# zengyan-97/X2-VLM

Hardware: AMD Instinct MI355X
Metric: image-text pairs/sec (fwd+bwd) X2VLM-base 224px bs=64/GPU (higher is better)
Workload: dtype bf16

## Files before the change

probes/nt_phase_times.py:

```python
import ctypes, importlib, os, sys
sys.path.insert(0, os.path.dirname(os.path.dirname(os.path.abspath(__file__))))
import torch
K = importlib.import_module("x2-vlm_amd.kernels")
lib = importlib.import_module("x2-vlm_amd._lib").lib()
assert hasattr(lib, "x2_probe_set_buffer"), "needs the probe build: X2VLM_HIP_LIB=probes/_probe/libx2vlm_hip_probe.so"
lib.x2_probe_set_buffer.argtypes, lib.x2_probe_set_buffer.restype = [ctypes.c_void_p], ctypes.c_int
dev = "cuda"
NSET = 12
SHAPES = [("vit qkv", 12608, 2304, 768, "bias"), ("vit dqkv", 12608, 768, 2304, "plain"), ("vit dfc1", 12608, 768, 3072, "plain"),
          ("vit fc2", 12608, 768, 3072, "lscale"), ("vit dproj", 12608, 768, 768, "plain"), ("fus xkv", 12608, 1536, 768, "bias"),
          ("vit fc1 (forced)", 12608, 3072, 768, "gelu"), ("vitL qkv", 18464, 3072, 1024, "bias"), ("vitL dfc1", 18464, 1024, 4096, "plain")]


def launch(kind, A, W, out, extra):
    if kind == "bias":
        K.gemm_nt(A, W, bias=extra["bias"], out=out)
    elif kind == "plain":
        K.gemm_nt(A, W, out=out)
    elif kind == "lscale":
        K.gemm_nt(A, W, bias=extra["bias"], gamma=extra["gamma"], resid=extra["resid"], out=out)
    elif kind == "gelu":
        K.gemm_nt(A, W, bias=extra["bias"], aux=extra["aux"], act=1, out=out)


for name, M, N, Kd, kind in SHAPES:
    f32 = kind == "lscale"
    As = [torch.randn(M, Kd, device=dev).bfloat16() for _ in range(NSET)]
    W = (torch.randn(N, Kd, device=dev) / Kd ** 0.5).bfloat16()
    outs = [torch.empty(M, N, device=dev, dtype=torch.float32 if f32 else torch.bfloat16) for _ in range(NSET)]
    extra = dict(bias=torch.randn(N, device=dev), gamma=torch.rand(N, device=dev), resid=torch.randn(M, N, device=dev) if f32 else None,
                 aux=torch.empty(M, N, device=dev, dtype=torch.bfloat16) if kind == "gelu" else None)
    lib.x2_tune(1, 3)
    nbuf = torch.zeros(4096 * 4, device=dev, dtype=torch.int64)
    for i in range(NSET):
        launch(kind, As[i], W, outs[i], extra)
    torch.cuda.synchronize()
    rows = []
    for rep in range(6):
        nbuf.zero_()
        lib.x2_probe_set_buffer(ctypes.c_void_p(nbuf.data_ptr()))
        launch(kind, As[rep % NSET], W, outs[rep % NSET], extra)
        torch.cuda.synchronize()
        lib.x2_probe_set_buffer(None)
        t = nbuf.view(-1, 4).cpu().double()
        t = t[t[:, 3] > 0] / 100.0
        t0 = t[:, 0].min()
        rows.append((t.shape[0], (t[:, 1] - t[:, 0]), (t[:, 2] - t[:, 1]), (t[:, 3] - t[:, 2]), float(t[:, 3].max() - t0),
                     float((t[:, 0] - t0).quantile(0.9))))
    lib.x2_tune(1, 0)
    n = rows[0][0]
    pro = torch.cat([r[1] for r in rows[1:]]); main = torch.cat([r[2] for r in rows[1:]]); epi = torch.cat([r[3] for r in rows[1:]])
    span = sum(r[4] for r in rows[1:]) / len(rows[1:])
    busy = float((pro.sum() + main.sum() + epi.sum()) / len(rows[1:])) / 256.0
    print("%-18s M=%6d N=%5d K=%5d %-6s | %4d wgs (%.2f rounds) | launch %6.1f us | prologue %5.2f (p90 %5.2f)  main %6.2f (p90 %6.2f)  epilogue %5.2f (p90 %5.2f) us"
          " | per CU: %.1f us busy = %.0f %% of the launch: prologue %.0f %%, main %.0f %%, epilogue %.0f %%; entry of the 90th percentile wg %+.1f us"
          % (name, M, N, Kd, kind, n, n / 256.0, span, pro.mean(), pro.quantile(0.9), main.mean(), main.quantile(0.9), epi.mean(), epi.quantile(0.9),
             busy, 100 * busy / span, 100 * float(pro.sum()) / float(pro.sum() + main.sum() + epi.sum()),
             100 * float(main.sum()) / float(pro.sum() + main.sum() + epi.sum()), 100 * float(epi.sum()) / float(pro.sum() + main.sum() + epi.sum()),
             rows[-1][5]))
```

x2-vlm_amd/csrc/gemm.hip:

```cpp
#include "x2_common.h"
#include <type_traits>

#define BM 128
#define BN 128
#define BK 64
#define TILE_BYTES (128 * 128)
#define STAGE_BYTES (2 * TILE_BYTES)
#define GEMM_LDS_BYTES (2 * STAGE_BYTES)

struct GemmNT {
  const bf16_t* A; const bf16_t* B; void* C;
  const float* bias; const float* gamma; const float* resid; bf16_t* aux;
  int M, N, K;
  int lda, ldb, ldc, ldr, ldaux;
  int act;
  int out_f32;
  int group_m;
  DropSpec drop;
  const uint32_t* drop_epoch;
  const float* rowscale;
  float* colsum;
  int dbg;
  int ksplit;
  const long* ce_labels;
  const float* ce_lse;
  const float* ce_g;
  const float* ce_stat;
  float* ce_part;
  float* ce_zlab;
  float ce_gscale;
  int ce_C;
  float* ce_sumz;
  float* ce_zign;
  long ce_ignore;
  float ce_ls;
  const float* ce_w;
};

__device__ __forceinline__ void tile_coords(int t, int tiles_m, int tiles_n, int gm, int& tm, int& tn) {
  const int gsz = gm * tiles_n, g = t / gsz, first = g * gm;
  const int rows = min(gm, tiles_m - first), r = t - g * gsz;
  tm = first + r % rows;
  tn = r / rows;
}

__device__ __forceinline__ void st16(void* p, u32x4 v, bool wt) {
  if (wt) asm volatile("global_store_dwordx4 %0, %1, off sc1\n\ts_nop 1" ::"v"(p), "v"(v) : "memory");
  else *reinterpret_cast<u32x4*>(p) = v;
}

#ifdef X2_PROBE
#define NT_DBG(p, bit) (((p).dbg & (bit)) != 0)
static __device__ unsigned long long* g_nt_probe = nullptr;
#define NT_STAMP(i) do { if (g_nt_probe && threadIdx.x == 0) g_nt_probe[(size_t)blockIdx.x * 4 + (i)] = wall_clock64(); } while (0)
#define NT_ABL_DECL(p) const bool abl_dma_ = NT_DBG(p, 32), abl_rd_ = NT_DBG(p, 64), abl_mm_ = NT_DBG(p, 128); bool rd_ = true
#define NT_ABL_NO_DMA(kt) if (abl_dma_ && (kt) >= 2) return
#define NT_ABL_NO_READ() if (!rd_) return
#define NT_ABL_NO_MFMA() if (abl_mm_) return
#define NT_ABL_STEP(kt) if (abl_rd_ && (kt) > 0) rd_ = false
#else
#define NT_ABL_DECL(p)
#define NT_ABL_NO_DMA(kt)
#define NT_ABL_NO_READ()
#define NT_ABL_NO_MFMA()
#define NT_ABL_STEP(kt)
#define NT_DBG(p, bit) false
#define NT_STAMP(i) do { } while (0)
#endif
typedef __attribute__((ext_vector_type(16))) float f32x16;
template <int TM>
__device__ __forceinline__ void epi_stage_half(f32x4 (&acc)[TM][4], int half, bool full, float* stg, int lane) {
  const int frow = lane & 15, fg = lane >> 4;
#pragma unroll
  for (int ii = 0; ii < 2; ++ii)
#pragma unroll
    for (int j = 0; j < 4; ++j)
      if (full || ii == 0) *reinterpret_cast<f32x4*>(stg + (ii * 16 + frow) * 68 + j * 16 + fg * 4) = acc[full ? half * 2 + ii : half * 2][j];
}
template <int RT>
__device__ __forceinline__ void epi_stage_half(f32x16 (&acc)[RT][2], int half, bool, float* stg, int lane) {
  const int row = lane & 31, h = lane >> 5;
#pragma unroll
  for (int tj = 0; tj < 2; ++tj)
#pragma unroll
    for (int g = 0; g < 4; ++g)
      *reinterpret_cast<f32x4*>(stg + row * 68 + tj * 32 + g * 8 + h * 4) =
          f32x4{acc[half][tj][4 * g], acc[half][tj][4 * g + 1], acc[half][tj][4 * g + 2], acc[half][tj][4 * g + 3]};
}
template <int V> struct EpiTraits {
  static constexpr bool generic = V == 4;
  static constexpr int act = V == 2 ? 1 : (V == 3 || V == 10) ? 2 : 0;
  static constexpr bool out_f32 = V == 1 || V == 5 || V == 6 || V == 7;
  static constexpr bool resid = V == 5 || V == 6;
  static constexpr bool scale = V == 6;
  static constexpr bool aux0 = false;
  static constexpr bool drop = V == 5;
  static constexpr bool colsum = false;
  static constexpr bool colparts = V == 10;
};
template <int TM, int VAR, class Acc>
__device__ __forceinline__ void nt_epilogue(const GemmNT& p, Acc& acc, char* smem, int wave, int lane, int mw0, int nw0, int prow = 0) {
  using E = EpiTraits<VAR>;
  const int act = E::generic ? p.act : E::act;
  const bool out_f32 = E::generic ? p.out_f32 != 0 : E::out_f32;
  const bool has_resid = E::generic ? p.resid != nullptr : E::resid;
  const bool has_scale = E::generic ? (p.gamma != nullptr || p.rowscale != nullptr) : E::scale;
  const bool has_aux0 = E::generic ? (p.act == 0 && p.aux != nullptr) : E::aux0;
  const bool has_drop = (E::generic || E::drop) ? p.drop.thr16 != 0 : false;
  const bool has_colsum = E::generic ? p.colsum != nullptr : (E::colsum && p.colsum != nullptr);
  float* stg = reinterpret_cast<float*>(smem) + wave * (32 * 68);
  const int er = lane >> 3, ec = (lane & 7) * 8;
  const int n = nw0 + ec;
  const bool nok = n < p.N;
  float bb[8], gg[8];
#pragma unroll
  for (int e = 0; e < 8; ++e) { bb[e] = 0.f; gg[e] = 1.f; }
  if (nok && p.bias) { const float4 b0 = *reinterpret_cast<const float4*>(p.bias + n), b1 = *reinterpret_cast<const float4*>(p.bias + n + 4);
    bb[0] = b0.x; bb[1] = b0.y; bb[2] = b0.z; bb[3] = b0.w; bb[4] = b1.x; bb[5] = b1.y; bb[6] = b1.z; bb[7] = b1.w; }
  if (nok && has_scale && p.gamma) { const float4 g0 = *reinterpret_cast<const float4*>(p.gamma + n), g1 = *reinterpret_cast<const float4*>(p.gamma + n + 4);
    gg[0] = g0.x; gg[1] = g0.y; gg[2] = g0.z; gg[3] = g0.w; gg[4] = g1.x; gg[5] = g1.y; gg[6] = g1.z; gg[7] = g1.w; }
  float cs[8] = {0.f, 0.f, 0.f, 0.f, 0.f, 0.f, 0.f, 0.f};
  const bool wt = NT_DBG(p, 16);
  const DropSpec drop_ = drop_at_epoch(p.drop, p.drop_epoch);
#pragma unroll
  for (int half = 0; half < (TM + 1) / 2; ++half) {
    const bool full = half * 2 + 1 < TM;
    float4 r0[4], r1[4];
    u32x4 pre[4];
    const int nc = nok ? n : 0;
    if (has_resid) {
#pragma unroll
      for (int rr = 0; rr < 4; ++rr) {
        if (!full && rr >= 2) continue;
        const int mc = min(mw0 + half * 32 + rr * 8 + er, p.M - 1);
        r0[rr] = *reinterpret_cast<const float4*>(p.resid + (size_t)mc * p.ldr + nc);
        r1[rr] = *reinterpret_cast<const float4*>(p.resid + (size_t)mc * p.ldr + nc + 4);
      }
    }
    if (act == 2) {
#pragma unroll
      for (int rr = 0; rr < 4; ++rr) {
        if (!full && rr >= 2) continue;
        const int mc = min(mw0 + half * 32 + rr * 8 + er, p.M - 1);
        pre[rr] = *reinterpret_cast<const u32x4*>(p.aux + (size_t)mc * p.ldaux + nc);
      }
    }
    epi_stage_half(acc, half, full, stg, lane);
#pragma unroll
    for (int rr = 0; rr < 4; ++rr) {
      if (!full && rr >= 2) continue;
      const int row = rr * 8 + er;
      const int m = mw0 + half * 32 + row;
      const float4 a0 = *reinterpret_cast<const float4*>(stg + row * 68 + ec), a1 = *reinterpret_cast<const float4*>(stg + row * 68 + ec + 4);
      if (m >= p.M || !nok) continue;
      float v[8] = {a0.x + bb[0], a0.y + bb[1], a0.z + bb[2], a0.w + bb[3], a1.x + bb[4], a1.y + bb[5], a1.z + bb[6], a1.w + bb[7]};
      if constexpr (VAR == 8) {
        const long lab = p.ce_labels[m];
        float mx = -INFINITY;
#pragma unroll
        for (int e = 0; e < 8; ++e) mx = n + e < p.ce_C ? fmaxf(mx, v[e]) : mx;
        mx = fmaxf(mx, __shfl_xor(mx, 1, 64)); mx = fmaxf(mx, __shfl_xor(mx, 2, 64)); mx = fmaxf(mx, __shfl_xor(mx, 4, 64));
        float se = 0.f;
#pragma unroll
        for (int e = 0; e < 8; ++e) {
          se += n + e < p.ce_C ? __expf(v[e] - mx) : 0.f;
          if ((long)(n + e) == lab) p.ce_zlab[m] = v[e];
        }
        se += __shfl_xor(se, 1, 64); se += __shfl_xor(se, 2, 64); se += __shfl_xor(se, 4, 64);
        if ((lane & 7) == 0) *reinterpret_cast<float2*>(p.ce_part + ((size_t)m * (p.N >> 6) + (nw0 >> 6)) * 2) = float2{mx, se};
        continue;
      }
      if constexpr (VAR == 11) {
        const long lab = p.ce_labels[m];
        float mx = -INFINITY, sz = 0.f;
#pragma unroll
        for (int e = 0; e < 8; ++e) { mx = n + e < p.ce_C ? fmaxf(mx, v[e]) : mx; sz += n + e < p.ce_C ? v[e] : 0.f; }
        mx = fmaxf(mx, __shfl_xor(mx, 1, 64)); mx = fmaxf(mx, __shfl_xor(mx, 2, 64)); mx = fmaxf(mx, __shfl_xor(mx, 4, 64));
        sz += __shfl_xor(sz, 1, 64); sz += __shfl_xor(sz, 2, 64); sz += __shfl_xor(sz, 4, 64);
        float se = 0.f;
#pragma unroll
        for (int e = 0; e < 8; ++e) {
          se += n + e < p.ce_C ? __expf(v[e] - mx) : 0.f;
          if ((long)(n + e) == lab) p.ce_zlab[m] = v[e];
          if ((long)(n + e) == p.ce_ignore) p.ce_zign[m] = v[e];
        }
        se += __shfl_xor(se, 1, 64); se += __shfl_xor(se, 2, 64); se += __shfl_xor(se, 4, 64);
        if ((lane & 7) == 0) {
          *reinterpret_cast<float2*>(p.ce_part + ((size_t)m * (p.N >> 6) + (nw0 >> 6)) * 2) = float2{mx, se};
          p.ce_sumz[(size_t)m * (p.N >> 6) + (nw0 >> 6)] = sz;
        }
        continue;
      }
      if constexpr (VAR == 12) {
        const long lab = p.ce_labels[m];
        const bool live = lab >= 0 && lab != p.ce_ignore;
        const float conf = 1.f - p.ce_ls, sm = p.ce_ls / (float)(p.ce_C - 2), qsum = conf + sm * (float)(p.ce_C - 2);
        const float sc = live ? p.ce_gscale * p.ce_g[0] * p.ce_w[m] / (p.ce_stat[1] + 1e-5f) : 0.f, l = p.ce_lse[m];
#pragma unroll
        for (int e = 0; e < 8; ++e) {
          const long c = n + e;
          const float q = c == lab ? conf : (c == p.ce_ignore ? 0.f : sm);
          v[e] = c < p.ce_C ? (qsum * __expf(v[e] - l) - q) * sc : 0.f;
        }
        st16(reinterpret_cast<bf16_t*>(p.C) + (size_t)m * p.ldc + n,
             u32x4{pack_bf16(v[0], v[1]), pack_bf16(v[2], v[3]), pack_bf16(v[4], v[5]), pack_bf16(v[6], v[7])}, false);
        continue;
      }
      if constexpr (VAR == 9) {
        const long lab = p.ce_labels[m];
        const float sc = lab >= 0 ? p.ce_gscale * p.ce_g[0] / p.ce_stat[1] : 0.f, l = p.ce_lse[m];
#pragma unroll
        for (int e = 0; e < 8; ++e) v[e] = n + e < p.ce_C ? (__expf(v[e] - l) - ((long)(n + e) == lab ? 1.f : 0.f)) * sc : 0.f;
        st16(reinterpret_cast<bf16_t*>(p.C) + (size_t)m * p.ldc + n,
             u32x4{pack_bf16(v[0], v[1]), pack_bf16(v[2], v[3]), pack_bf16(v[4], v[5]), pack_bf16(v[6], v[7])}, false);
        continue;
      }
      if (act == 1) {
        st16(p.aux + (size_t)m * p.ldaux + n, u32x4{pack_bf16(v[0], v[1]), pack_bf16(v[2], v[3]), pack_bf16(v[4], v[5]), pack_bf16(v[6], v[7])}, wt);
#pragma unroll
        for (int r = 0; r < 8; ++r) v[r] = gelu_f(v[r]);
      } else if (act == 2) {
#pragma unroll
        for (int r = 0; r < 4; ++r) { v[2 * r] *= dgelu_f(bf_lo(pre[rr][r])); v[2 * r + 1] *= dgelu_f(bf_hi(pre[rr][r])); }
      } else if (has_aux0) {
        st16(p.aux + (size_t)m * p.ldaux + n, u32x4{pack_bf16(v[0], v[1]), pack_bf16(v[2], v[3]), pack_bf16(v[4], v[5]), pack_bf16(v[6], v[7])}, wt);
      }
      if (has_drop) {
        float dm[4];
        drop_mul4(drop_, (uint32_t)m * (uint32_t)p.N + (uint32_t)n, dm);
        v[0] *= dm[0]; v[1] *= dm[1]; v[2] *= dm[2]; v[3] *= dm[3];
        drop_mul4(drop_, (uint32_t)m * (uint32_t)p.N + (uint32_t)n + 4u, dm);
        v[4] *= dm[0]; v[5] *= dm[1]; v[6] *= dm[2]; v[7] *= dm[3];
      }
      if (has_scale) {
        const float rs_ = p.rowscale ? p.rowscale[m] : 1.f;
#pragma unroll
        for (int r = 0; r < 8; ++r) v[r] *= gg[r] * rs_;
      }
      if (has_resid) {
        v[0] += r0[rr].x; v[1] += r0[rr].y; v[2] += r0[rr].z; v[3] += r0[rr].w;
        v[4] += r1[rr].x; v[5] += r1[rr].y; v[6] += r1[rr].z; v[7] += r1[rr].w;
      }
      if (has_colsum || E::colparts) {
#pragma unroll
        for (int r = 0; r < 8; ++r) cs[r] += v[r];
      }
      if (out_f32) {
        float* c = reinterpret_cast<float*>(p.C) + (size_t)m * p.ldc + n;
        st16(c, u32x4{__float_as_uint(v[0]), __float_as_uint(v[1]), __float_as_uint(v[2]), __float_as_uint(v[3])}, wt);
        st16(c + 4, u32x4{__float_as_uint(v[4]), __float_as_uint(v[5]), __float_as_uint(v[6]), __float_as_uint(v[7])}, wt);
      } else {
        st16(reinterpret_cast<bf16_t*>(p.C) + (size_t)m * p.ldc + n,
             u32x4{pack_bf16(v[0], v[1]), pack_bf16(v[2], v[3]), pack_bf16(v[4], v[5]), pack_bf16(v[6], v[7])}, wt);
      }
    }
  }
  if constexpr (E::colparts) {
#pragma unroll
    for (int e = 0; e < 8; ++e) { cs[e] += __shfl_xor(cs[e], 8, 64); cs[e] += __shfl_xor(cs[e], 16, 64); cs[e] += __shfl_xor(cs[e], 32, 64); }
    if (er == 0 && nok) {
      float* dst = p.colsum + (size_t)prow * p.N + n;
      *reinterpret_cast<float4*>(dst) = float4{cs[0], cs[1], cs[2], cs[3]};
      *reinterpret_cast<float4*>(dst + 4) = float4{cs[4], cs[5], cs[6], cs[7]};
    }
  }
  if (has_colsum) {
#pragma unroll
    for (int e = 0; e < 8; ++e) { cs[e] += __shfl_xor(cs[e], 8, 64); cs[e] += __shfl_xor(cs[e], 16, 64); cs[e] += __shfl_xor(cs[e], 32, 64); }
    if (er == 0 && nok) {
#pragma unroll
      for (int e = 0; e < 8; ++e) atomicAdd(p.colsum + n + e, cs[e]);
    }
  }
}

template <int TM, int VAR, class Acc>
__device__ __forceinline__ void nt_epilogue_f4(const GemmNT& p, Acc& acc, char* smem, int wave, int lane, int mw0, int nw0) {
  using E = EpiTraits<VAR>;
  static_assert(!E::generic && E::out_f32 && E::act == 0 && VAR <= 6, "nt_epilogue_f4: feature sets 1, 5, 6");
  const bool has_drop = E::drop ? p.drop.thr16 != 0 : false;
  float* stg = reinterpret_cast<float*>(smem) + wave * (32 * 68);
  const int er = lane >> 4, ec = (lane & 15) * 4;
  const int n = nw0 + ec;
  const bool nok = n < p.N;
  float bb[4] = {0.f, 0.f, 0.f, 0.f}, gg[4] = {1.f, 1.f, 1.f, 1.f};
  if (nok && p.bias) { const float4 b0 = *reinterpret_cast<const float4*>(p.bias + n); bb[0] = b0.x; bb[1] = b0.y; bb[2] = b0.z; bb[3] = b0.w; }
  if (E::scale && nok && p.gamma) { const float4 g0 = *reinterpret_cast<const float4*>(p.gamma + n); gg[0] = g0.x; gg[1] = g0.y; gg[2] = g0.z; gg[3] = g0.w; }
  const DropSpec drop_ = drop_at_epoch(p.drop, p.drop_epoch);
#pragma unroll
  for (int half = 0; half < (TM + 1) / 2; ++half) {
    const bool full = half * 2 + 1 < TM;
    float4 rs[4][2];
    const int nc = nok ? n : 0;
    if (E::resid) {
#pragma unroll
      for (int rr = 0; rr < 4; ++rr) {
        if (!full && rr >= 2) continue;
#pragma unroll
        for (int h = 0; h < 2; ++h) {
          const int mc = min(mw0 + half * 32 + rr * 8 + h * 4 + er, p.M - 1);
          rs[rr][h] = *reinterpret_cast<const float4*>(p.resid + (size_t)mc * p.ldr + nc);
        }
      }
    }
    epi_stage_half(acc, half, full, stg, lane);
#pragma unroll
    for (int rr = 0; rr < 4; ++rr) {
      if (!full && rr >= 2) continue;
#pragma unroll
      for (int h = 0; h < 2; ++h) {
        const int row = rr * 8 + h * 4 + er;
        const int m = mw0 + half * 32 + row;
        const float4 a0 = *reinterpret_cast<const float4*>(stg + row * 68 + ec);
        if (m >= p.M || !nok) continue;
        float v[4] = {a0.x + bb[0], a0.y + bb[1], a0.z + bb[2], a0.w + bb[3]};
        if (has_drop) {
          float dm[4];
          drop_mul4(drop_, (uint32_t)m * (uint32_t)p.N + (uint32_t)n, dm);
          v[0] *= dm[0]; v[1] *= dm[1]; v[2] *= dm[2]; v[3] *= dm[3];
        }
        if (E::scale) {
          const float rs_ = p.rowscale ? p.rowscale[m] : 1.f;
#pragma unroll
          for (int r = 0; r < 4; ++r) v[r] *= gg[r] * rs_;
        }
        if (E::resid) { v[0] += rs[rr][h].x; v[1] += rs[rr][h].y; v[2] += rs[rr][h].z; v[3] += rs[rr][h].w; }
        st16(reinterpret_cast<float*>(p.C) + (size_t)m * p.ldc + n,
             u32x4{__float_as_uint(v[0]), __float_as_uint(v[1]), __float_as_uint(v[2]), __float_as_uint(v[3])}, false);
      }
    }
  }
}

template <int TM, int VAR, bool F4 = false>
__global__ __launch_bounds__(256, 2) void gemm_nt_kernel(GemmNT p) {
  constexpr int BMT = 32 * TM;
  if constexpr (VAR == 7) {
    const int koff = blockIdx.y * p.ksplit;
    p.A += koff; p.B += koff;
    p.K = min(p.ksplit, p.K - koff);
    p.C = reinterpret_cast<float*>(p.C) + (size_t)blockIdx.y * p.M * p.ldc;
  }
  constexpr int A_BYTES = BMT * 128, STG = A_BYTES + TILE_BYTES;
  extern __shared__ __attribute__((aligned(16))) char smem[];
  const int tid = threadIdx.x, lane = tid & 63;
  const int wave = __builtin_amdgcn_readfirstlane(tid >> 6);
  const int wm = wave >> 1, wn = wave & 1;
  const int tiles_n = (p.N + BN - 1) / BN, tiles_m = (p.M + BMT - 1) / BMT;
  int tm, tn;
  tile_coords(xcd_remap(blockIdx.x, gridDim.x), tiles_m, tiles_n, p.group_m, tm, tn);
  const int m0 = tm * BMT, n0 = tn * BN;

  const bf16_t* srcA[TM]; const bf16_t* srcB[4];
#pragma unroll
  for (int i = 0; i < TM; ++i) {
    const int q = i * 256 + tid, row = q >> 3, c = (q & 7) ^ (row & 7);
// ... 280 lines not shown
        fb[ks][jh * 2 + j] = lds_read_b128(buf + offB + (jh * 2 + j) * 2048 + (uint32_t)(((ks * 4 + fg) ^ fsw) << 4));
  };
  auto readBx = [&](uint32_t buf) {
#pragma unroll
    for (int ks = 0; ks < 2; ++ks)
#pragma unroll
      for (int j = 0; j < 2; ++j)
        fbx[ks][j] = lds_read_b128(buf + offB + j * 2048 + (uint32_t)(((ks * 4 + fg) ^ fsw) << 4));
  };
  auto quad = [&](auto hi_, auto jh_) {
    constexpr bool hi = decltype(hi_)::value;
    constexpr int jh = decltype(jh_)::value, first = hi ? TH : 0, count = hi ? TMW - TH : TH;
#pragma unroll
    for (int ks = 0; ks < 2; ++ks)
#pragma unroll
      for (int i = 0; i < count; ++i)
#pragma unroll
        for (int j = 0; j < 2; ++j)
          acc[first + i][jh * 2 + j] = __builtin_amdgcn_mfma_f32_16x16x32_bf16(fb[ks][jh * 2 + j], (PIPE && hi) ? fah[ks][i] : fa[ks][i],
                                                                               acc[first + i][jh * 2 + j], 0, 0, 0);
  };
  using LO = std::false_type; using HI = std::true_type;
#define N3_FENCE() __builtin_amdgcn_sched_barrier(0)
  int rs = 0, ws = 2;
  auto ptile = [&](int kt, auto n1_, auto n2_, auto first_) {
    constexpr bool n1 = decltype(n1_)::value, n2 = decltype(n2_)::value, first = decltype(first_)::value;
    const uint32_t buf = lds0 + (uint32_t)(rs * N3_STAGE), nbuf = lds0 + (uint32_t)((rs == 2 ? 0 : rs + 1) * N3_STAGE);
    if constexpr (!first) {
      asm volatile("s_waitcnt lgkmcnt(0)" ::: "memory");
      N3_FENCE();
#pragma unroll
      for (int ks = 0; ks < 2; ++ks) { fb[ks][0] = fbx[ks][0]; fb[ks][1] = fbx[ks][1]; }
    }
    if constexpr (n2) issue(ws, kt + 2, S0{});
    N3_FENCE();
    quad(LO{}, S0{}); N3_FENCE();
    readA(buf, HI{});
    if constexpr (n2) issue(ws, kt + 2, S1{});
    N3_FENCE();
    quad(LO{}, S1{}); N3_FENCE();
    if constexpr (n2) issue(ws, kt + 2, S2{});
    N3_FENCE();
    asm volatile("s_waitcnt lgkmcnt(0)" ::: "memory");
    N3_FENCE();
    quad(HI{}, S1{}); N3_FENCE();
    if constexpr (n1) {
      if constexpr (n2) asm volatile("s_waitcnt vmcnt(4)\n\ts_barrier" ::: "memory");
      else asm volatile("s_waitcnt vmcnt(0)\n\ts_barrier" ::: "memory");
      N3_FENCE();
      readA(nbuf, LO{}); readB(nbuf, 1); readBx(nbuf);
    }
    if constexpr (n2) issue(ws, kt + 2, S3{});
    N3_FENCE();
    quad(HI{}, S0{}); N3_FENCE();
    rs = rs == 2 ? 0 : rs + 1;
    ws = ws == 2 ? 0 : ws + 1;
  };
  auto ktile = [&](int kt, auto n1_, auto n2_) {
    constexpr bool n1 = decltype(n1_)::value, n2 = decltype(n2_)::value;
    const uint32_t buf = lds0 + (uint32_t)(rs * N3_STAGE);
    readA(buf, LO{}); readB(buf, 0); readB(buf, 1);
    if constexpr (n2) issue(ws, kt + 2, S0{});
    N3_FENCE();
    quad(LO{}, S0{}); N3_FENCE();
    if constexpr (n2) issue(ws, kt + 2, S1{});
    N3_FENCE();
    quad(LO{}, S1{}); N3_FENCE();
    readA(buf, HI{});
    if constexpr (n2) issue(ws, kt + 2, S2{});
    N3_FENCE();
    quad(HI{}, S1{}); N3_FENCE();
    if constexpr (n2) issue(ws, kt + 2, S3{});
    N3_FENCE();
    quad(HI{}, S0{}); N3_FENCE();
    if constexpr (n1) {
      if constexpr (n2) asm volatile("s_waitcnt vmcnt(6) lgkmcnt(0)\n\ts_barrier" ::: "memory");
      else asm volatile("s_waitcnt vmcnt(0) lgkmcnt(0)\n\ts_barrier" ::: "memory");
      N3_FENCE();
    }
    rs = rs == 2 ? 0 : rs + 1;
    ws = ws == 2 ? 0 : ws + 1;
  };
  const int nk = p.K / BK;
  issue(0, 0, S0{}); issue(0, 0, S1{}); issue(0, 0, S2{}); issue(0, 0, S3{});
  if (nk > 1) {
    issue(1, 1, S0{}); issue(1, 1, S1{}); issue(1, 1, S2{}); issue(1, 1, S3{});
    asm volatile("s_waitcnt vmcnt(6)\n\ts_barrier" ::: "memory");
  } else {
    asm volatile("s_waitcnt vmcnt(0)\n\ts_barrier" ::: "memory");
  }
  int kt = 0;
  if constexpr (PIPE) {
    readA(lds0, LO{}); readB(lds0, 0); readB(lds0, 1);
    asm volatile("s_waitcnt lgkmcnt(0)" ::: "memory");
    N3_FENCE();
    if (nk >= 3) { ptile(0, std::true_type{}, std::true_type{}, std::true_type{}); kt = 1; }
    else if (nk == 2) { ptile(0, std::true_type{}, std::false_type{}, std::true_type{}); kt = 1; }
    else { ptile(0, std::false_type{}, std::false_type{}, std::true_type{}); kt = 1; }
    for (; kt + 2 < nk; ++kt) ptile(kt, std::true_type{}, std::true_type{}, std::false_type{});
    if (kt + 1 < nk) { ptile(kt, std::true_type{}, std::false_type{}, std::false_type{}); ++kt; }
    if (kt < nk) ptile(kt, std::false_type{}, std::false_type{}, std::false_type{});
  } else {
    for (; kt + 2 < nk; ++kt) ktile(kt, std::true_type{}, std::true_type{});
    if (kt + 1 < nk) { ktile(kt, std::true_type{}, std::false_type{}); ++kt; }
    ktile(kt, std::false_type{}, std::false_type{});
  }
#undef N3_FENCE
  asm volatile("s_waitcnt lgkmcnt(0)\n\ts_barrier" ::: "memory");
  nt_epilogue<TMW, VAR>(p, acc, smem, wave, lane, m0 + wr * HROWS, n0 + wc * 64);
}

#define PP_BHALF 16384
template <int N_> __device__ __forceinline__ void pp_wait_vm() { asm volatile("s_waitcnt vmcnt(%0)" ::"n"(N_) : "memory"); }
template <int RT0, int RT1, int VAR, int NST>
__global__ __launch_bounds__(512) void gemm_nt_pp_kernel(GemmNT p) {
  constexpr int BMT = 32 * (RT0 + RT1);
  constexpr int A0_BYTES = RT0 * 4096, A1_BYTES = RT1 * 4096, STAGE = A0_BYTES + A1_BYTES + 2 * PP_BHALF;
  extern __shared__ __attribute__((aligned(16))) char smem[];
  const int tid = threadIdx.x, lane = tid & 63;
  const int wave = __builtin_amdgcn_readfirstlane(tid >> 6);
  const int wr = wave >> 2, wc = wave & 3;
  const int tiles_n = (p.N + 255) / 256, tiles_m = (p.M + BMT - 1) / BMT;
  int tm, tn;
  tile_coords(xcd_remap(blockIdx.x, gridDim.x), tiles_m, tiles_n, p.group_m, tm, tn);
  const int m0 = tm * BMT, n0 = tn * 256;
  const uint32_t lds0 = lds_addr(smem);
  const int drow = wc * 8 + (lane >> 3), dchunk = (lane & 7) ^ ((wc & 1) * 4 + (lane >> 4));
  uint32_t foff[4];
#pragma unroll
  for (int ks = 0; ks < 4; ++ks) foff[ks] = (uint32_t)((lane & 31) * 128 + (((ks * 2 + (lane >> 5)) ^ ((lane >> 1) & 7)) << 4));
  const uint32_t boff = (uint32_t)(A0_BYTES + A1_BYTES + (wc >> 1) * PP_BHALF + (wc & 1) * 8192);
  const int nk = p.K / BK;
  NT_ABL_DECL(p);
  NT_STAMP(0);

  auto run = [&](auto rt_, auto first_) {
    constexpr int RT = decltype(rt_)::value;
    constexpr bool FIRST = decltype(first_)::value;
    const uint32_t aoff = FIRST ? 0u : (uint32_t)A0_BYTES;
    f32x16 acc[RT][2];
#pragma unroll
    for (int i = 0; i < RT; ++i)
#pragma unroll
      for (int j = 0; j < 2; ++j)
#pragma unroll
        for (int e = 0; e < 16; ++e) acc[i][j][e] = 0.f;
    bf16x8 fa[RT][4], fb[2][4];
    const __amdgpu_buffer_rsrc_t rs = FIRST
        ? __builtin_amdgcn_make_buffer_rsrc((void*)p.B, 0, (int)(((size_t)(p.N - 1) * p.ldb + p.K) * 2), 0x00020000)
        : __builtin_amdgcn_make_buffer_rsrc((void*)p.A, 0, (int)(((size_t)(p.M - 1) * p.lda + p.K) * 2), 0x00020000);
    const int ld = FIRST ? p.ldb : p.lda;
    const uint32_t v0 = (uint32_t)(((size_t)((FIRST ? n0 : m0) + drow) * ld + dchunk * 8) * 2);
    const uint32_t step32 = (uint32_t)ld * 64u;
    auto dma = [&](int kt, int stage, int region_bytes_off, int row32_first, auto count_) {
      constexpr int CNT = decltype(count_)::value;
      NT_ABL_NO_DMA(kt + 1);
#pragma unroll
      for (int q = 0; q < CNT; ++q)
        __builtin_amdgcn_raw_ptr_buffer_load_lds(rs, (__attribute__((address_space(3))) void*)(smem + stage * STAGE + region_bytes_off + q * 4096 + wc * 1024),
                                                 16, v0 + (uint32_t)(row32_first + q) * step32, kt * 128, 0, 0);
    };
    using C4 = std::integral_constant<int, 4>; using CR0 = std::integral_constant<int, RT0>; using CR1 = std::integral_constant<int, RT1>;
    auto reads = [&](uint32_t sb) {
      NT_ABL_NO_READ();
#pragma unroll
      for (int ks = 0; ks < 4; ++ks)
#pragma unroll
        for (int j = 0; j < 2; ++j) fb[j][ks] = lds_read_b128(sb + boff + foff[ks] + j * 4096);
#pragma unroll
      for (int ks = 0; ks < 4; ++ks)
#pragma unroll
        for (int i = 0; i < RT; ++i) fa[i][ks] = lds_read_b128(sb + aoff + foff[ks] + i * 4096);
    };
    auto mfmas = [&]() {
      NT_ABL_NO_MFMA();
      __builtin_amdgcn_s_setprio(1);
#pragma unroll
      for (int ks = 0; ks < 4; ++ks)
#pragma unroll
        for (int i = 0; i < RT; ++i)
#pragma unroll
          for (int j = 0; j < 2; ++j)
            acc[i][j] = __builtin_amdgcn_mfma_f32_32x32x16_bf16(fb[j][ks], fa[i][ks], acc[i][j], 0, 0, 0);
      __builtin_amdgcn_s_setprio(0);
    };
#define PP_FENCE() __builtin_amdgcn_sched_barrier(0)
#define PP_BARRIER() do { PP_FENCE(); asm volatile("s_barrier" ::: "memory"); PP_FENCE(); } while (0)
    if constexpr (NST == 3) {
      constexpr int MINE = FIRST ? 8 : RT0 + RT1;
      auto request = [&](int kt, int stage) {
        if constexpr (FIRST) { dma(kt, stage, A0_BYTES + A1_BYTES, 0, C4{}); dma(kt, stage, A0_BYTES + A1_BYTES + PP_BHALF, 4, C4{}); }
        else { dma(kt, stage, 0, 0, CR0{}); dma(kt, stage, A0_BYTES, RT0, CR1{}); }
// ... 7 lines not shown
      for (int t = 0; t < nk; ++t) {
        const uint32_t sb = lds0 + (uint32_t)(rs * STAGE);
        NT_ABL_STEP(t);
        const bool more = t + 2 < nk;
        if (more) request(t + 2, ws);
        reads(sb);
        PP_FENCE();
        if constexpr (!FIRST) { if (more) pp_wait_vm<MINE>(); else pp_wait_vm<0>(); }
        asm volatile("s_waitcnt lgkmcnt(0)" ::: "memory");
        PP_BARRIER();
        mfmas();
        PP_FENCE();
        if constexpr (FIRST) { if (more) pp_wait_vm<MINE>(); else pp_wait_vm<0>(); }
        PP_BARRIER();
        rs = rs == 2 ? 0 : rs + 1;
        ws = ws == 2 ? 0 : ws + 1;
      }
    } else {
      if constexpr (FIRST) {
        dma(0, 0, A0_BYTES + A1_BYTES, 0, C4{}); dma(0, 0, A0_BYTES + A1_BYTES + PP_BHALF, 4, C4{});
        pp_wait_vm<0>();
      } else {
        dma(0, 0, A0_BYTES, RT0, CR1{}); dma(0, 0, 0, 0, CR0{});
        if (nk > 1) { dma(1, 1, 0, 0, CR0{}); pp_wait_vm<RT0>(); } else pp_wait_vm<0>();
      }
      PP_BARRIER();
      if constexpr (!FIRST) PP_BARRIER();
      NT_STAMP(1);
      for (int t = 0; t < nk; ++t) {
        const int s_ = t & 1;
        const uint32_t sb = lds0 + (uint32_t)(s_ * STAGE);
        NT_ABL_STEP(t);
        if constexpr (FIRST) {
          if (t + 1 < nk) { dma(t + 1, s_ ^ 1, A0_BYTES + A1_BYTES, 0, C4{}); dma(t + 1, s_ ^ 1, A0_BYTES + A1_BYTES + PP_BHALF, 4, C4{}); }
          reads(sb);
          asm volatile("s_waitcnt lgkmcnt(0)" ::: "memory");
          PP_BARRIER();
          mfmas();
          PP_FENCE();
          pp_wait_vm<0>();
          PP_BARRIER();
        } else {
          int mode = 0;
          if (t + 2 < nk) { dma(t + 1, s_ ^ 1, A0_BYTES, RT0, CR1{}); dma(t + 2, s_, 0, 0, CR0{}); mode = 2; }
          else if (t + 1 < nk) { dma(t + 1, s_ ^ 1, A0_BYTES, RT0, CR1{}); mode = 1; }
          reads(sb);
          PP_FENCE();
          if (mode == 2) pp_wait_vm<RT0 + RT1>(); else if (mode == 1) pp_wait_vm<RT1>(); else pp_wait_vm<0>();
          asm volatile("s_waitcnt lgkmcnt(0)" ::: "memory");
          PP_BARRIER();
          mfmas();
          PP_FENCE();
          if (mode == 2) pp_wait_vm<RT0>(); else pp_wait_vm<0>();
          PP_BARRIER();
        }
      }
    }
    if constexpr (FIRST) PP_BARRIER();
    NT_STAMP(2);
#undef PP_BARRIER
#undef PP_FENCE
    const int mw0 = m0 + (FIRST ? 0 : RT0 * 32), nw0 = n0 + wc * 64;
    if constexpr (EpiTraits<VAR>::out_f32 && VAR <= 6) nt_epilogue_f4<2 * RT, VAR>(p, acc, smem, wave, lane, mw0, nw0);
    else nt_epilogue<2 * RT, VAR>(p, acc, smem, wave, lane, mw0, nw0);
#ifdef X2_PROBE
    asm volatile("s_waitcnt vmcnt(0)" ::: "memory");
    NT_STAMP(3);
#endif
  };
  if (wr == 0) run(std::integral_constant<int, RT0>{}, std::true_type{});
  else run(std::integral_constant<int, RT1>{}, std::false_type{});
}

static int g_tune[8] = {0, 0, 0, 0, 0, 0, 0, 0};
static int g_tune_x[8] = {0, 0, 0, 0, 0, 0, 0, 0};
extern "C" int x2_device_cus(void);
static int x2_cus() {
  static int n = 0;
  if (n <= 0) { n = x2_device_cus(); if (n <= 0) n = 256; }
  const int left = n - g_tune_x[4];
  return left >= 16 ? left : 16;
}
extern "C" int x2_tune(int key, int value) {
  if (key >= 9 && key <= 15) {
    X2_REQUIRE(key != 12 || value >= 0, "x2_tune: reserved compute units = %d", value);
    g_tune_x[key - 8] = value;
    return X2_OK;
  }
  X2_REQUIRE(key >= 0 && key < 8, "x2_tune: no key %d", key);
#ifndef X2_PROBE
  X2_REQUIRE(key != 2 || value == 0, "x2_tune: NT ablation bits (key 2, value %d) exist in -DX2_PROBE builds only", value);
#endif
  g_tune[key] = value;
  return X2_OK;
}
#ifdef X2_PROBE
extern "C" int x2_probe_set_buffer(void* buf) {
  unsigned long long* b = (unsigned long long*)buf;
  return hipMemcpyToSymbol(HIP_SYMBOL(g_nt_probe), &b, sizeof(b)) == hipSuccess ? X2_OK : X2_ERR_LAUNCH;
}
#endif
extern "C" int x2_tune_get(int key) {
  if (key >= 9 && key <= 15) return g_tune_x[key - 8];
  if (key < 0 || key >= 8) return -1;
  return g_tune[key];
}

static int nt256_plan(int M, int N, double* eff) {
  const int cus = x2_cus(), tiles_n = (N + 255) / 256;
  const double ideal = (double)M * N / (512.0 * 256.0 * cus);
  int best = 8; double best_cost = 1e30;
  for (int t = 8; t >= 5; --t) {
    const long tiles = (long)((M + 32 * t - 1) / (32 * t)) * tiles_n;
    const double cost = (double)((tiles + cus - 1) / cus) * t / 16.0;
    if (cost < best_cost - 1e-9) { best_cost = cost; best = t; }
  }
  if (eff) *eff = ideal / best_cost;
  return best;
}
template <int TMW, int V>
static void launch_nt256(const GemmNT& p, hipStream_t stream) {
  static bool raised = false;
  if (!raised) {
    (void)hipFuncSetAttribute(reinterpret_cast<const void*>(gemm_nt256_kernel<TMW, V>), hipFuncAttributeMaxDynamicSharedMemorySize, N2_LDS_BYTES);
    raised = true;
  }
  const int tiles = ((p.M + 32 * TMW - 1) / (32 * TMW)) * ((p.N + 255) / 256);
  hipLaunchKernelGGL((gemm_nt256_kernel<TMW, V>), dim3(tiles), dim3(512), N2_LDS_BYTES, stream, p);
}
template <int V>
static void launch_nt256s3(const GemmNT& p, hipStream_t stream) {
  static bool raised = false;
  if (!raised) {
    (void)hipFuncSetAttribute(reinterpret_cast<const void*>(gemm_nt256s3_kernel<V, true>), hipFuncAttributeMaxDynamicSharedMemorySize, N3_LDS_BYTES);
    (void)hipFuncSetAttribute(reinterpret_cast<const void*>(gemm_nt256s3_kernel<V, false>), hipFuncAttributeMaxDynamicSharedMemorySize, N3_LDS_BYTES);
    raised = true;
  }
  const int tiles = ((p.M + 159) / 160) * ((p.N + 255) / 256);
  if (g_tune_x[2] == 2) hipLaunchKernelGGL((gemm_nt256s3_kernel<V, false>), dim3(tiles), dim3(512), N3_LDS_BYTES, stream, p);
  else hipLaunchKernelGGL((gemm_nt256s3_kernel<V, true>), dim3(tiles), dim3(512), N3_LDS_BYTES, stream, p);
}
template <int V>
static void launch_nt256_h(const GemmNT& p, int tmw, hipStream_t stream) {
  switch (tmw) {
    case 5: if (g_tune_x[2] == 1) launch_nt256<5, V>(p, stream); else launch_nt256s3<V>(p, stream); break;
    case 6: launch_nt256<6, V>(p, stream); break;
    case 7: launch_nt256<7, V>(p, stream); break;
    default: launch_nt256<8, V>(p, stream); break;
  }
}

template <int RT0, int RT1, int V, int NST>
static void launch_nt_pp(const GemmNT& p, hipStream_t stream) {
  constexpr int lds = NST * ((RT0 + RT1) * 4096 + 2 * PP_BHALF);
  static bool raised = false;
  if (!raised) {
    (void)hipFuncSetAttribute(reinterpret_cast<const void*>(gemm_nt_pp_kernel<RT0, RT1, V, NST>), hipFuncAttributeMaxDynamicSharedMemorySize, lds);
    raised = true;
  }
  constexpr int BMT = 32 * (RT0 + RT1);
  const int tiles = ((p.M + BMT - 1) / BMT) * ((p.N + 255) / 256);
  hipLaunchKernelGGL((gemm_nt_pp_kernel<RT0, RT1, V, NST>), dim3(tiles), dim3(512), lds, stream, p);
}
template <int V>
static void launch_nt_pp_h(const GemmNT& p, int h, hipStream_t stream) {
  switch (h) {
    case 3: launch_nt_pp<1, 2, V, 3>(p, stream); break;
    case 4: if (g_tune_x[2] == 1) launch_nt_pp<2, 2, V, 2>(p, stream); else launch_nt_pp<2, 2, V, 3>(p, stream); break;
    case 5: if (g_tune_x[2] == 1) launch_nt_pp<2, 3, V, 2>(p, stream); else launch_nt_pp<2, 3, V, 3>(p, stream); break;
    default: launch_nt_pp<3, 3, V, 2>(p, stream); break;
  }
}

template <int TM, int V, bool F4>
static void launch_nt(const GemmNT& p, int tiles, hipStream_t stream) {
  constexpr int lds = 2 * (32 * TM * 128 + TILE_BYTES);
  static bool raised = false;
  if (lds > 65536 && !raised) {
    (void)hipFuncSetAttribute(reinterpret_cast<const void*>(gemm_nt_kernel<TM, V, F4>), hipFuncAttributeMaxDynamicSharedMemorySize, lds);
    raised = true;
  }
  hipLaunchKernelGGL((gemm_nt_kernel<TM, V, F4>), dim3(tiles), dim3(256), lds, stream, p);
}

extern "C" int x2_gemm_nt(const void* A, const void* B, void* C, int M, int N, int K, int lda, int ldb, int ldc,
                          const float* bias, const float* gamma, const float* resid, int ldr, void* aux, int ldaux,
                          int act, int out_f32, unsigned drop_thr16, unsigned drop_seed, float drop_scale, const unsigned* drop_epoch,
                          const float* rowscale, float* colsum, void* stream) {
  X2_REQUIRE(M > 0 && N > 0 && K > 0, "x2_gemm_nt: empty problem M=%d N=%d K=%d", M, N, K);
  X2_REQUIRE(drop_thr16 < 65536u, "x2_gemm_nt: drop_thr16=%u", drop_thr16);
  X2_REQUIRE(K % BK == 0, "x2_gemm_nt: K=%d must be a multiple of %d", K, BK);
  X2_REQUIRE(N % 8 == 0, "x2_gemm_nt: N=%d must be a multiple of 8", N);
  X2_REQUIRE(lda % 8 == 0 && ldb % 8 == 0 && ldc % 8 == 0, "x2_gemm_nt: leading dims must keep 16-byte rows");
  X2_REQUIRE(act == 0 || aux, "x2_gemm_nt: act=%d needs aux", act);
  X2_REQUIRE((!resid || ldr % 4 == 0) && (!aux || ldaux % 8 == 0), "x2_gemm_nt: ldr/ldaux alignment");
  GemmNT p{(const bf16_t*)A, (const bf16_t*)B, C, bias, gamma, resid, (bf16_t*)aux, M, N, K, lda, ldb, ldc, ldr, ldaux, act, out_f32,
           g_tune[0] > 0 ? g_tune[0] : 8, DropSpec{drop_thr16, drop_seed, drop_scale}, drop_epoch, rowscale, colsum, g_tune[2], 0};
  int var = 4;
  {
    const bool plain = !gamma && !rowscale && !drop_thr16 && !colsum;
    if (g_tune[6] == 1) var = 4;
    else if (act == 1 && !out_f32 && !resid && plain) var = 2;
    else if (act == 2 && !out_f32 && !resid && plain) var = 3;
    else if (act == 0 && !aux && !resid && plain) var = out_f32 ? 1 : 0;
    else if (act == 0 && !aux && resid && out_f32 && !gamma && !rowscale && !colsum) var = 5;
    else if (act == 0 && !aux && resid && out_f32 && gamma && !drop_thr16 && !colsum) var = 6;
  }
  double eff256 = 0.0;
  int tmw = nt256_plan(M, N, &eff256);
  if (g_tune[3] >= 5 && g_tune[3] <= 8) tmw = g_tune[3];
  const bool light = var == 0 || var == 1;
  bool auto256 = (light || K >= 2048) && eff256 * 100.0 >= (g_tune_x[1] > 0 ? g_tune_x[1] : 80) && !(resid && M < 8192);
  if (g_tune_x[3] != 1) {
    if ((var == 5 || var == 6) && M >= 8192 && eff256 * 100.0 >= (g_tune_x[1] > 0 ? g_tune_x[1] : 80)) auto256 = true;
    if (var == 2 && eff256 * 100.0 >= 90.0) auto256 = true;
  }
  const bool use256 = var != 4 && N % 8 == 0 && (g_tune[1] == 3 || ((g_tune[1] == 0 || g_tune[1] == 4) && g_tune[3] == 0 && auto256));
  const bool pp_ok = var != 4 && ((size_t)(M - 1) * lda + K) * 2 < (1ull << 31) && ((size_t)(N - 1) * ldb + K) * 2 < (1ull << 31);
  int pp_h = 0;
  if (g_tune_x[7] >= 3 && g_tune_x[7] <= 6) pp_h = g_tune_x[7];
  else if (g_tune_x[7] == 0 && g_tune[1] == 0 && g_tune[3] == 0 && !use256 && K >= 2048 && (var == 0 || var == 1 || var == 5)) {
    const int cus = x2_cus(), tn256 = (N + 255) / 256;
    for (int h = 3; h <= 4 && !pp_h; ++h) {
      const int tiles = ((M + 32 * h - 1) / (32 * h)) * tn256;
      if (tiles <= cus && tiles * 10 >= cus * 7) pp_h = h;
    }
// ... 528 lines not shown
```

Baseline: 2953.

## Add persistent 160x256 NT GEMM kernel overlapping next tile loads with epilogue

Adds a persistent variant of the 3-stage 256-wide NT GEMM. It launches at most one workgroup per CU and loops over tiles, prefetching the next tile's first K stages while the current tile drains and runs its epilogue. The epilogue staging area is relocated into free pipeline stages so it does not clash with the prefetched data. The kernel is selected by default when tmw=5, the tile count exceeds the CU count, K<=1024 and 32-bit offsets fit. This targets launch tail and prologue/epilogue bubbles, at the cost of more complex LDS stage bookkeeping and a fixed tile order across CUs.

After: 2954 (median of 4 runs). No clear change (+0.0%).

```diff
diff --git a/probes/nt_phase_times.py b/probes/nt_phase_times.py
--- a/probes/nt_phase_times.py
+++ b/probes/nt_phase_times.py
@@ -9,7 +9,10 @@
 NSET = 12
 SHAPES = [("vit qkv", 12608, 2304, 768, "bias"), ("vit dqkv", 12608, 768, 2304, "plain"), ("vit dfc1", 12608, 768, 3072, "plain"),
           ("vit fc2", 12608, 768, 3072, "lscale"), ("vit dproj", 12608, 768, 768, "plain"), ("fus xkv", 12608, 1536, 768, "bias"),
-          ("vit fc1 (forced)", 12608, 3072, 768, "gelu"), ("vitL qkv", 18464, 3072, 1024, "bias"), ("vitL dfc1", 18464, 1024, 4096, "plain")]
+          ("vit fc1 (forced)", 12608, 3072, 768, "gelu"), ("vitL qkv", 18464, 3072, 1024, "bias"), ("vitL dfc1", 18464, 1024, 4096, "plain"),
+          ("vit dfc2 (forced)", 12608, 3072, 768, "dgelu"), ("txt ffn1 (forced)", 7680, 3072, 768, "gelu")]
+if os.environ.get("NT_SHAPES"):
+    SHAPES = [s_ for s_ in SHAPES if s_[0] in os.environ["NT_SHAPES"].split(",")]
 
 
 def launch(kind, A, W, out, extra):
@@ -21,6 +24,8 @@
         K.gemm_nt(A, W, bias=extra["bias"], gamma=extra["gamma"], resid=extra["resid"], out=out)
     elif kind == "gelu":
         K.gemm_nt(A, W, bias=extra["bias"], aux=extra["aux"], act=1, out=out)
+    elif kind == "dgelu":
+        K.gemm_nt(A, W, aux=extra["aux"], act=2, out=out)
 
 
 for name, M, N, Kd, kind in SHAPES:
@@ -29,7 +34,7 @@
     W = (torch.randn(N, Kd, device=dev) / Kd ** 0.5).bfloat16()
     outs = [torch.empty(M, N, device=dev, dtype=torch.float32 if f32 else torch.bfloat16) for _ in range(NSET)]
     extra = dict(bias=torch.randn(N, device=dev), gamma=torch.rand(N, device=dev), resid=torch.randn(M, N, device=dev) if f32 else None,
-                 aux=torch.empty(M, N, device=dev, dtype=torch.bfloat16) if kind == "gelu" else None)
+                 aux=torch.randn(M, N, device=dev).bfloat16() if kind in ("gelu", "dgelu") else None)
     lib.x2_tune(1, 3)
     nbuf = torch.zeros(4096 * 4, device=dev, dtype=torch.int64)
     for i in range(NSET):
diff --git a/x2-vlm_amd/csrc/gemm.hip b/x2-vlm_amd/csrc/gemm.hip
--- a/x2-vlm_amd/csrc/gemm.hip
+++ b/x2-vlm_amd/csrc/gemm.hip
@@ -99,7 +99,7 @@
   static constexpr bool colparts = V == 10;
 };
 template <int TM, int VAR, class Acc>
-__device__ __forceinline__ void nt_epilogue(const GemmNT& p, Acc& acc, char* smem, int wave, int lane, int mw0, int nw0, int prow = 0) {
+__device__ __forceinline__ void nt_epilogue_at(const GemmNT& p, Acc& acc, float* stg, int lane, int mw0, int nw0, int prow = 0) {
   using E = EpiTraits<VAR>;
   const int act = E::generic ? p.act : E::act;
   const bool out_f32 = E::generic ? p.out_f32 != 0 : E::out_f32;
@@ -108,7 +108,6 @@
   const bool has_aux0 = E::generic ? (p.act == 0 && p.aux != nullptr) : E::aux0;
   const bool has_drop = (E::generic || E::drop) ? p.drop.thr16 != 0 : false;
   const bool has_colsum = E::generic ? p.colsum != nullptr : (E::colsum && p.colsum != nullptr);
-  float* stg = reinterpret_cast<float*>(smem) + wave * (32 * 68);
   const int er = lane >> 3, ec = (lane & 7) * 8;
   const int n = nw0 + ec;
   const bool nok = n < p.N;
@@ -272,6 +271,10 @@
       for (int e = 0; e < 8; ++e) atomicAdd(p.colsum + n + e, cs[e]);
     }
   }
+}
+template <int TM, int VAR, class Acc>
+__device__ __forceinline__ void nt_epilogue(const GemmNT& p, Acc& acc, char* smem, int wave, int lane, int mw0, int nw0, int prow = 0) {
+  nt_epilogue_at<TM, VAR>(p, acc, reinterpret_cast<float*>(smem) + wave * (32 * 68), lane, mw0, nw0, prow);
 }
 
 template <int TM, int VAR, class Acc>
@@ -718,6 +721,7 @@
     ws = ws == 2 ? 0 : ws + 1;
   };
   const int nk = p.K / BK;
+  NT_STAMP(0);
   issue(0, 0, S0{}); issue(0, 0, S1{}); issue(0, 0, S2{}); issue(0, 0, S3{});
   if (nk > 1) {
     issue(1, 1, S0{}); issue(1, 1, S1{}); issue(1, 1, S2{}); issue(1, 1, S3{});
@@ -725,6 +729,7 @@
   } else {
     asm volatile("s_waitcnt vmcnt(0)\n\ts_barrier" ::: "memory");
   }
+  NT_STAMP(1);
   int kt = 0;
   if constexpr (PIPE) {
     readA(lds0, LO{}); readB(lds0, 0); readB(lds0, 1);
@@ -743,7 +748,176 @@
   }
 #undef N3_FENCE
   asm volatile("s_waitcnt lgkmcnt(0)\n\ts_barrier" ::: "memory");
+  NT_STAMP(2);
   nt_epilogue<TMW, VAR>(p, acc, smem, wave, lane, m0 + wr * HROWS, n0 + wc * 64);
+#ifdef X2_PROBE
+  asm volatile("s_waitcnt vmcnt(0)" ::: "memory");
+  NT_STAMP(3);
+#endif
+}
+
+template <int VAR>
+__global__ __launch_bounds__(512) void gemm_nt256p_kernel(GemmNT p, int tiles) {
+  constexpr int TMW = 5, BMT = 32 * TMW, HROWS = 16 * TMW, TH = 3;
+  extern __shared__ __attribute__((aligned(16))) char smem[];
+  const int tid = threadIdx.x, lane = tid & 63;
+  const int wave = __builtin_amdgcn_readfirstlane(tid >> 6);
+  const int wr = wave >> 2, wc = wave & 3;
+  const int tiles_n = (p.N + 255) / 256, tiles_m = (p.M + BMT - 1) / BMT;
+  uint32_t srcA[2][2], srcB[2][2];
+  int am0 = 0, an0 = 0;
+  auto aim = [&](int t) {
+    int tm, tn;
+    tile_coords(xcd_remap(t, tiles), tiles_m, tiles_n, p.group_m, tm, tn);
+    am0 = tm * BMT; an0 = tn * 256;
+#pragma unroll
+    for (int h = 0; h < 2; ++h)
+#pragma unroll
+      for (int i = 0; i < 2; ++i) {
+        const int q = i * 512 + tid, row = q >> 3, c = (q & 7) ^ (row & 7);
+        int ra = am0 + h * HROWS + (row < HROWS ? row : HROWS - 1); ra = ra < p.M ? ra : p.M - 1;
+        int rb = an0 + h * 128 + row; rb = rb < p.N ? rb : p.N - 1;
+        srcA[h][i] = (uint32_t)ra * (uint32_t)p.lda + (uint32_t)(c * 8);
+        srcB[h][i] = (uint32_t)rb * (uint32_t)p.ldb + (uint32_t)(c * 8);
+      }
+  };
+  const bool a2 = wave < 2 * TMW - 8;
+  auto issue = [&](int stage, int kt, auto slot) {
+    constexpr int S = decltype(slot)::value;
+    char* base = smem + stage * N3_STAGE + (S < 2 ? S * N3_A_HALF : 2 * N3_A_HALF + (S - 2) * N2_HALF) + wave * 1024;
+    if constexpr (S < 2) {
+      const bf16_t* a = p.A + (size_t)kt * BK;
+      glds16(a + srcA[S][0], base);
+      if (a2) glds16(a + srcA[S][1], base + 8192);
+    } else {
+      const bf16_t* b = p.B + (size_t)kt * BK;
+      glds16(b + srcB[S - 2][0], base);
+      glds16(b + srcB[S - 2][1], base + 8192);
+    }
+  };
+  using S0 = std::integral_constant<int, 0>; using S1 = std::integral_constant<int, 1>;
+  using S2 = std::integral_constant<int, 2>; using S3 = std::integral_constant<int, 3>;
+  f32x4 acc[TMW][4];
+  const uint32_t lds0 = lds_addr(smem);
+  const int frow = lane & 15, fg = lane >> 4, fsw = lane & 7;
+  const uint32_t offA = (uint32_t)(wr * N3_A_HALF + frow * 128);
+  const uint32_t offB = (uint32_t)(2 * N3_A_HALF + (wc >> 1) * N2_HALF + ((wc & 1) * 64 + frow) * 128);
+  bf16x8 fa[2][TH], fb[2][4], fah[2][TMW - TH], fbx[2][2];
+  auto readA = [&](uint32_t buf, auto hi_) {
+    constexpr bool hi = decltype(hi_)::value;
+    constexpr int first = hi ? TH : 0, count = hi ? TMW - TH : TH;
+#pragma unroll
+    for (int ks = 0; ks < 2; ++ks)
+#pragma unroll
+      for (int i = 0; i < count; ++i) {
+        const bf16x8 v = lds_read_b128(buf + offA + (first + i) * 2048 + (uint32_t)(((ks * 4 + fg) ^ fsw) << 4));
+        if constexpr (hi) fah[ks][i] = v; else fa[ks][i] = v;
+      }
+  };
+  auto readB = [&](uint32_t buf, int jh) {
+#pragma unroll
+    for (int ks = 0; ks < 2; ++ks)
+#pragma unroll
+      for (int j = 0; j < 2; ++j)
+        fb[ks][jh * 2 + j] = lds_read_b128(buf + offB + (jh * 2 + j) * 2048 + (uint32_t)(((ks * 4 + fg) ^ fsw) << 4));
+  };
+  auto readBx = [&](uint32_t buf) {
+#pragma unroll
+    for (int ks = 0; ks < 2; ++ks)
+#pragma unroll
+      for (int j = 0; j < 2; ++j)
+        fbx[ks][j] = lds_read_b128(buf + offB + j * 2048 + (uint32_t)(((ks * 4 + fg) ^ fsw) << 4));
+  };
+  auto quad = [&](auto hi_, auto jh_) {
+    constexpr bool hi = decltype(hi_)::value;
+    constexpr int jh = decltype(jh_)::value, first = hi ? TH : 0, count = hi ? TMW - TH : TH;
+#pragma unroll
+    for (int ks = 0; ks < 2; ++ks)
+#pragma unroll
+      for (int i = 0; i < count; ++i)
+#pragma unroll
+        for (int j = 0; j < 2; ++j)
+          acc[first + i][jh * 2 + j] = __builtin_amdgcn_mfma_f32_16x16x32_bf16(fb[ks][jh * 2 + j], hi ? fah[ks][i] : fa[ks][i],
+                                                                               acc[first + i][jh * 2 + j], 0, 0, 0);
+  };
+  using LO = std::false_type; using HI = std::true_type;
+  using T = std::true_type; using F = std::false_type;
+#define N3_FENCE() __builtin_amdgcn_sched_barrier(0)
+  int rs = 0, ws = 2;
+  auto ptile = [&](int kreq, bool req, auto n1_, auto n2_, auto first_) {
+    constexpr bool n1 = decltype(n1_)::value, n2 = decltype(n2_)::value, first = decltype(first_)::value;
+    const uint32_t buf = lds0 + (uint32_t)(rs * N3_STAGE), nbuf = lds0 + (uint32_t)((rs == 2 ? 0 : rs + 1) * N3_STAGE);
+    if constexpr (!first) {
+      asm volatile("s_waitcnt lgkmcnt(0)" ::: "memory");
+      N3_FENCE();
+#pragma unroll
+      for (int ks = 0; ks < 2; ++ks) { fb[ks][0] = fbx[ks][0]; fb[ks][1] = fbx[ks][1]; }
+    }
+    if constexpr (n2) { if (req) issue(ws, kreq, S0{}); }
+    N3_FENCE();
+    quad(LO{}, S0{}); N3_FENCE();
+    readA(buf, HI{});
+    if constexpr (n2) { if (req) issue(ws, kreq, S1{}); }
+    N3_FENCE();
+    quad(LO{}, S1{}); N3_FENCE();
+    if constexpr (n2) { if (req) issue(ws, kreq, S2{}); }
+    N3_FENCE();
+    asm volatile("s_waitcnt lgkmcnt(0)" ::: "memory");
+    N3_FENCE();
+    quad(HI{}, S1{}); N3_FENCE();
+    if constexpr (n1) {
+      if (n2 && req) asm volatile("s_waitcnt vmcnt(4)\n\ts_barrier" ::: "memory");
+      else asm volatile("s_waitcnt vmcnt(0)\n\ts_barrier" ::: "memory");
+      N3_FENCE();
+      readA(nbuf, LO{}); readB(nbuf, 1); readBx(nbuf);
+    }
+    if constexpr (n2) { if (req) issue(ws, kreq, S3{}); }
+    N3_FENCE();
+    quad(HI{}, S0{}); N3_FENCE();
+    rs = rs == 2 ? 0 : rs + 1;
+    ws = ws == 2 ? 0 : ws + 1;
+  };
+  const int nk = p.K / BK;
+  int t = blockIdx.x;
+  aim(t);
+  issue(0, 0, S0{}); issue(0, 0, S1{}); issue(0, 0, S2{}); issue(0, 0, S3{});
+  issue(1, 1, S0{}); issue(1, 1, S1{}); issue(1, 1, S2{}); issue(1, 1, S3{});
+  asm volatile("s_waitcnt vmcnt(6)\n\ts_barrier" ::: "memory");
+  for (;;) {
+    const int m0 = am0, n0 = an0;
+    const int tnext = t + (int)gridDim.x;
+    const bool more = tnext < tiles;
+#pragma unroll
+    for (int i = 0; i < TMW; ++i)
+#pragma unroll
+      for (int j = 0; j < 4; ++j) acc[i][j] = f32x4{0.f, 0.f, 0.f, 0.f};
+    {
+      const uint32_t buf = lds0 + (uint32_t)(rs * N3_STAGE);
+      readA(buf, LO{}); readB(buf, 0); readB(buf, 1);
+      asm volatile("s_waitcnt lgkmcnt(0)" ::: "memory");
+      N3_FENCE();
+    }
+    ptile(2, true, T{}, T{}, T{});
+    int kt = 1;
+    for (; kt + 2 < nk; ++kt) ptile(kt + 2, true, T{}, T{}, F{});
+    if (more) aim(tnext);
+    ptile(0, more, T{}, T{}, F{});
+    ptile(0, false, F{}, F{}, F{});
+    asm volatile("s_waitcnt vmcnt(0) lgkmcnt(0)\n\ts_barrier" ::: "memory");
+    N3_FENCE();
+    {
+      const int sst = wave < 6 ? ws : (rs == 2 ? 0 : rs + 1);
+      float* stg = reinterpret_cast<float*>(smem + sst * N3_STAGE + (wave < 6 ? wave : wave - 6) * (32 * 68 * 4));
+      nt_epilogue_at<TMW, VAR>(p, acc, stg, lane, m0 + wr * HROWS, n0 + wc * 64);
+    }
+    if (!more) break;
+    t = tnext;
+    asm volatile("s_waitcnt lgkmcnt(0)\n\ts_barrier" ::: "memory");
+    N3_FENCE();
+    const int s1 = rs == 2 ? 0 : rs + 1;
+    issue(s1, 1, S0{}); issue(s1, 1, S1{}); issue(s1, 1, S2{}); issue(s1, 1, S3{});
+  }
+#undef N3_FENCE
 }
 
 #define PP_BHALF 16384
@@ -917,8 +1091,9 @@
   return left >= 16 ? left : 16;
 }
 extern "C" int x2_tune(int key, int value) {
-  if (key >= 9 && key <= 15) {
+  if (key >= 8 && key <= 15) {
     X2_REQUIRE(key != 12 || value >= 0, "x2_tune: reserved compute units = %d", value);
+    X2_REQUIRE(key != 8 || (value >= 0 && value <= 2), "x2_tune: persistent NT kernel (key 8) = %d", value);
     g_tune_x[key - 8] = value;
     return X2_OK;
   }
@@ -936,7 +1111,7 @@
 }
 #endif
 extern "C" int x2_tune_get(int key) {
-  if (key >= 9 && key <= 15) return g_tune_x[key - 8];
+  if (key >= 8 && key <= 15) return g_tune_x[key - 8];
   if (key < 0 || key >= 8) return -1;
   return g_tune[key];
 }
@@ -976,7 +1151,25 @@
   else hipLaunchKernelGGL((gemm_nt256s3_kernel<V, true>), dim3(tiles), dim3(512), N3_LDS_BYTES, stream, p);
 }
 template <int V>
+static void launch_nt256p(const GemmNT& p, hipStream_t stream) {
+  static bool raised = false;
+  if (!raised) {
+    (void)hipFuncSetAttribute(reinterpret_cast<const void*>(gemm_nt256p_kernel<V>), hipFuncAttributeMaxDynamicSharedMemorySize, N3_LDS_BYTES);
+    raised = true;
+  }
+  const int tiles = ((p.M + 159) / 160) * ((p.N + 255) / 256), cus = x2_cus();
+  hipLaunchKernelGGL((gemm_nt256p_kernel<V>), dim3(tiles < cus ? tiles : cus), dim3(512), N3_LDS_BYTES, stream, p, tiles);
+}
+static bool nt256_persistent(const GemmNT& p, int tmw) {
+  if (tmw != 5 || g_tune_x[2] != 0 || g_tune_x[0] == 1 || p.K < 3 * BK) return false;
+  if ((size_t)(p.M - 1) * p.lda + p.K >= (1ull << 31) || (size_t)(p.N - 1) * p.ldb + p.K >= (1ull << 31)) return false;
+  if (g_tune_x[0] == 2) return true;
+  const int tiles = ((p.M + 159) / 160) * ((p.N + 255) / 256);
+  return tiles > x2_cus() && p.K <= 1024;
+}
+template <int V>
 static void launch_nt256_h(const GemmNT& p, int tmw, hipStream_t stream) {
+  if (nt256_persistent(p, tmw)) { launch_nt256p<V>(p, stream); return; }
   switch (tmw) {
     case 5: if (g_tune_x[2] == 1) launch_nt256<5, V>(p, stream); else launch_nt256s3<V>(p, stream); break;
     case 6: launch_nt256<6, V>(p, stream); break;
```
